# dkohlsdorf/audio_pattern_discovery

Hardware: AMD Instinct MI355X
Metric: DTW cell-updates/sec (whole node) (higher is better)
Workload: dtype f32

## Files before the change

### audio_pattern_discovery_amd/csrc/apd_api.hip

```cpp
#include <algorithm>
#include <cmath>
#include <cstdio>
#include <cstdlib>
#include <cstring>
#include <map>
#include <new>

#include "apd_internal.h"

using namespace apd;

namespace {

int ensure_ws(apd_context *ctx, void **p, size_t *have, size_t need)
{
    APD_AFFINITY(ctx, "workspace allocation");
    if (*have >= need && *p) return APD_OK;
    if (*p) { HIP_TRY(ctx, hipFree(*p)); *p = nullptr; *have = 0; }
    HIP_TRY(ctx, hipMalloc(p, need));
    *have = need;
    return APD_OK;
}

uint32_t tiles_side(uint32_t n_seq) { return (n_seq + kTile - 1) / kTile; }
// ... 43 lines not shown
    return hipSetDevice(ctx->device);
}
bool affinity_ok(const apd_context *ctx, const char *where)
{
    int dev = -1;
    const bool ok = tl_bound_context == ctx && hipGetDevice(&dev) == hipSuccess && dev == ctx->device;
    if (!ok) {
        const_cast<apd_context *>(ctx)->last_error = std::string("APD_DEBUG_AFFINITY: ") + where + " on a thread bound to " +
            (tl_bound_context == ctx ? "this context but HIP device " + std::to_string(dev) :
             tl_bound_context ? "another context (device " + std::to_string(tl_bound_context->device) + ")" : "no context") +
            ", expected device " + std::to_string(ctx->device);
        std::fprintf(stderr, "[apd] %s\n", ctx->last_error.c_str());
    }
    return ok;
}
}


extern "C" const char *apd_status_string(int s)
{
    switch (s) {
        case APD_OK: return "ok";
        case APD_ERR_INVALID_ARG: return "invalid argument";
        case APD_ERR_NO_DEVICE: return "no gfx950 HIP device";
        case APD_ERR_HIP: return "HIP runtime error";
        case APD_ERR_OOM: return "out of device memory";
        case APD_ERR_EMPTY_SEQUENCE: return "zero-length sequence (undefined in the reference, alignments.rs:120)";
        case APD_ERR_BAND_TOO_WIDE: return "warping band too wide for one wavefront";
        case APD_ERR_INDEX: return "percentile index out of range (the reference panics, numerics.rs:132)";
        case APD_ERR_UNSUPPORTED: return "unsupported";
        case APD_ERR_INCOMPLETE: return "a pair score was never written (launch cut short or skipped): NaN left in the output";
        case APD_ERR_COMM: return "RCCL error";
        default: return "unknown status";
    }
}

extern "C" int apd_create(int device, apd_context **out)
{
    if (!out) return APD_ERR_INVALID_ARG;
    *out = nullptr;
    int count = 0;
    if (hipGetDeviceCount(&count) != hipSuccess || count <= 0 || device < 0 || device >= count) return APD_ERR_NO_DEVICE;
    hipDeviceProp_t prop;
    if (hipGetDeviceProperties(&prop, device) != hipSuccess) return APD_ERR_NO_DEVICE;
    if (std::strncmp(prop.gcnArchName, "gfx950", 6) != 0) return APD_ERR_NO_DEVICE;
    apd_context *ctx = new (std::nothrow) apd_context();
    if (!ctx) return APD_ERR_OOM;
    ctx->device = device;
    if (bind_device(ctx) != hipSuccess || hipStreamCreateWithFlags(&ctx->stream, hipStreamNonBlocking) != hipSuccess) {
        delete ctx;
        return APD_ERR_HIP;
    }
    ctx->own_stream = true;
    if (hipMalloc((void **)&ctx->d_status, 64) != hipSuccess || hipMemset(ctx->d_status, 0, 64) != hipSuccess) {
        hipStreamDestroy(ctx->stream);
        delete ctx;
        return APD_ERR_OOM;
    }
    hipEventCreate(&ctx->ev0);
    hipEventCreate(&ctx->ev1);
    hipEventCreateWithFlags(&ctx->fork, hipEventDisableTiming);
    for (int k = 0; k < apd_context::kSideStreams; ++k) {
        hipStreamCreateWithFlags(&ctx->side[k], hipStreamNonBlocking);
        hipEventCreateWithFlags(&ctx->side_done[k], hipEventDisableTiming);
    }
    *out = ctx;
    return APD_OK;
}

static void release_batch_device_memory(apd_batch *b);

extern "C" int apd_destroy(apd_context *ctx)
{
    if (!ctx) return APD_ERR_INVALID_ARG;
    bind_device(ctx);
    hipStreamSynchronize(ctx->stream);
    if (ctx->pair_batch) { apd_batch_destroy(ctx->pair_batch); ctx->pair_batch = nullptr; }
    for (apd_batch *b : ctx->batches) { release_batch_device_memory(b); b->ctx = nullptr; }
    ctx->batches.clear();
    for (apd_comm *c : ctx->comms) apd::orphan_comm(c);
    ctx->comms.clear();
    for (apd_encoder *e : ctx->encoders) apd::orphan_encoder(e);
    ctx->encoders.clear();
    for (apd_cepstrum_plan *cp : ctx->cepstrum_plans) apd::orphan_cepstrum_plan(cp);
    ctx->cepstrum_plans.clear();
    for (void *p : ctx->buffers) hipFree(p);
    ctx->buffers.clear();
    if (ctx->ws_tiles) hipFree(ctx->ws_tiles);
    if (ctx->ws_slab) hipFree(ctx->ws_slab);
    if (ctx->ws_misc) hipFree(ctx->ws_misc);
    if (ctx->ws_gather) hipFree(ctx->ws_gather);
    if (ctx->d_status) hipFree(ctx->d_status);
    if (ctx->ev0) hipEventDestroy(ctx->ev0);
    if (ctx->ev1) hipEventDestroy(ctx->ev1);
    if (ctx->fork) hipEventDestroy(ctx->fork);
    for (int k = 0; k < apd_context::kSideStreams; ++k) {
        if (ctx->side[k]) { hipStreamSynchronize(ctx->side[k]); hipStreamDestroy(ctx->side[k]); }
        if (ctx->side_done[k]) hipEventDestroy(ctx->side_done[k]);
    }
    if (ctx->own_stream && ctx->stream) hipStreamDestroy(ctx->stream);
    delete ctx;
    return APD_OK;
}

extern "C" int apd_set_stream(apd_context *ctx, void *hip_stream)
{
// ... 296 lines not shown
extern "C" int apd_length_order(const uint64_t *offsets, uint32_t n_seq, uint32_t *order)
{
    if (!offsets || (n_seq && !order)) return APD_ERR_INVALID_ARG;
    std::vector<uint32_t> o;
    length_order(offsets, n_seq, o);
    std::copy(o.begin(), o.end(), order);
    return APD_OK;
}

extern "C" int apd_unpack_tiles_host(const uint64_t *offsets, uint32_t n_seq, uint32_t world, const float *gathered, float *out)
{
    if (!offsets || world == 0 || (n_seq && (!gathered || !out))) return APD_ERR_INVALID_ARG;
    std::vector<uint32_t> order;
    length_order(offsets, n_seq, order);
    const uint64_t slab = apd_slab_floats(n_seq, world);
    std::memset(out, 0, (size_t)n_seq * n_seq * sizeof(float));
    const uint32_t side = tiles_side(n_seq);
    uint64_t g = 0;
    for (uint32_t ta = 0; ta < side; ++ta)
        for (uint32_t tb = ta; tb < side; ++tb, ++g) {
            const float *t = gathered + (g % world) * slab + (g / world) * 2 * kSlotsPerTile;
            for (uint32_t sa = 0; sa < kTile; ++sa)
                for (uint32_t sb = 0; sb < kTile; ++sb) {
                    const uint32_t pa = ta * kTile + sa, pb = tb * kTile + sb;
                    if (pa < pb && pb < n_seq) {
                        const uint32_t a = order[pa], b = order[pb];
                        out[(uint64_t)a * n_seq + b] = t[sa * kTile + sb];
                        out[(uint64_t)b * n_seq + a] = t[kSlotsPerTile + sa * kTile + sb];
                    }
                }
        }
    return APD_OK;
}

static int check_lengths(const apd_batch *b)
{
    if (b->n_seq > 0 && b->min_len == 0) return APD_ERR_EMPTY_SEQUENCE;
    return APD_OK;
}

static int build_tile_plan(apd_context *ctx, const apd_batch *batch, const BandSpec &band, uint32_t rank, uint32_t world,
                           bool fast_ok, bool uniform_pen, bool fast_shift, apd_batch::TilePlan &plan_out)
{
    apd_batch::TilePlan plan;
    std::vector<uint2> tiles;
    rank_tile_list(batch->n_seq, rank, world, tiles);
    std::vector<uint4> flat;
    plan_tile_classes(batch->offsets, batch->n_seq, tiles, band, batch->dim, ctx->variant, fast_ok, uniform_pen, fast_shift,
                      plan.classes, flat);
    if (std::getenv("APD_DEBUG_PLAN"))
        for (const TileClass &tc : plan.classes)
            std::fprintf(stderr, "[apd] rank %u/%u: geometry %d: %u tiles, w_max %u, n_max %u\n", rank, world, tc.geom.encode(), tc.count,
                         tc.w_max, tc.n_max);
    HIP_TRY(ctx, hipMalloc((void **)&plan.d_tiles, std::max<size_t>(flat.size(), 1) * sizeof(uint4)));
    if (!flat.empty()) {
        hipError_t e = hipMemcpyAsync(plan.d_tiles, flat.data(), flat.size() * sizeof(uint4), hipMemcpyHostToDevice, ctx->stream);
        if (e == hipSuccess) e = hipStreamSynchronize(ctx->stream);
        if (e != hipSuccess) {
            hipFree(plan.d_tiles);
            ctx->last_error = std::string("tile plan upload: ") + hipGetErrorString(e);
            return APD_ERR_HIP;
        }
    }
    plan_out = std::move(plan);
    return APD_OK;
}

static int align_tiles_impl(apd_context *ctx, const apd_batch *batch, const BandSpec &band, uint32_t rank,
                            uint32_t world, float *d_slab)
{
    if (!ctx || !batch || !d_slab || world == 0 || rank >= world || batch->ctx != ctx) return APD_ERR_INVALID_ARG;
    int rc = check_lengths(batch);
    if (rc) return rc;
    HIP_TRY(ctx, bind_device(ctx));
    const bool pens_ok = (band.ins > 0.0f) && (band.del > 0.0f) && (band.mat > 0.0f) && (band.ins < INFINITY) &&
                         (band.del < INFINITY) && (band.mat < INFINITY);
    const bool static_fast = pens_ok && batch->frames_bytes != 0;
    bool nonfinite = false, device_select = false;
    if (static_fast) {
        const uint32_t band_ub = band.use_explicit ? band.explicit_band : host_band_from_pct(band.pct, batch->max_len);
        const uint32_t w_all = std::max(std::min(band_ub, batch->max_len), batch->max_len - batch->min_len) + 2;
        device_select = generic_fallback_fits(w_all) && apd_num_tiles(batch->n_seq) * kSlotsPerTile <= 0xFFFFFFFFull;
        if (!device_select) {
            rc = batch_nonfinite(ctx, batch, &nonfinite);
            if (rc) return rc;
        }
    }
    const bool fast_ok = static_fast && !nonfinite;
    const bool strict = ctx->distance_mode == 2;
    const bool uniform_pen = (band.ins == band.del) && (band.del == band.mat) && !strict;
    char keybuf[160];
    uint32_t pct_bits;
    std::memcpy(&pct_bits, &band.pct, sizeof(pct_bits));
    const bool fast_shift = band.ins == 1.0f && band.del == 1.0f && band.mat == 1.0f && ctx->distance_mode == 1 && batch->dim >= 8;
    std::snprintf(keybuf, sizeof(keybuf), "%u/%u/%08x/%u/%d/%d/%d/%d/%d", rank, world, pct_bits, band.explicit_band, band.use_explicit,
                  ctx->variant, (int)fast_ok, (int)uniform_pen, (int)fast_shift);
    auto cached = batch->tile_cache.find(keybuf);
    if (cached == batch->tile_cache.end()) {
        apd_batch::TilePlan fresh;
        rc = build_tile_plan(ctx, batch, band, rank, world, fast_ok, uniform_pen, fast_shift, fresh);
        if (rc) return rc;
        cached = batch->tile_cache.emplace(keybuf, std::move(fresh)).first;
    }
    const apd_batch::TilePlan &plan = cached->second;
    APD_AFFINITY(ctx, "alignment launches");
    HIP_TRY(ctx, hipMemsetAsync(d_slab, 0xFF, apd_slab_floats(batch->n_seq, world) * sizeof(float), ctx->stream));
    AlignLaunch L{};
    L.d_frames = batch->d_frames; L.frames_bytes = batch->frames_bytes; L.d_seq_off = batch->d_seq_off; L.d_seq_nmax = batch->d_seq_nmax;
    L.n_seq = batch->n_seq; L.dim = batch->dim; L.dpad = batch->dpad; L.band = band; L.d_slab = d_slab;
    L.variant = ctx->variant;
    L.hybrid = ctx->distance_mode == 1; L.strict = strict; L.tau = ctx->tau;
    L.d_nonfinite = device_select ? batch->d_flags : nullptr;
    if (ctx->timing) HIP_TRY(ctx, hipEventRecord(ctx->ev0, ctx->stream));
    const bool fan_out = plan.classes.size() > 1 && ctx->side[0] != nullptr;
    if (fan_out) {
        HIP_TRY(ctx, hipEventRecord(ctx->fork, ctx->stream));
        for (int k = 0; k < apd_context::kSideStreams; ++k) HIP_TRY(ctx, hipStreamWaitEvent(ctx->side[k], ctx->fork, 0));
    }
    int rc_launch = APD_OK;
    size_t ci = 0;
    for (const TileClass &tc : plan.classes) {
        L.d_tiles = plan.d_tiles + tc.first; L.n_tiles = tc.count; L.w_max = tc.w_max; L.n_max = tc.n_max;
        if (ctx->drop_tiles) L.n_tiles -= std::min(L.n_tiles, ctx->drop_tiles);
        int status = APD_OK;
        hipStream_t s = fan_out ? ctx->side[ci++ % apd_context::kSideStreams] : ctx->stream;
        hipError_t e = launch_align(L, tc.geom, s, ctx->last_error, &status);
        if (e != hipSuccess) { ctx->last_error = std::string("launch_align: ") + hipGetErrorString(e); rc_launch = APD_ERR_HIP; break; }
        if (status != APD_OK) { rc_launch = status; break; }
    }
    if (fan_out)
        for (int k = 0; k < apd_context::kSideStreams; ++k) {
            HIP_TRY(ctx, hipEventRecord(ctx->side_done[k], ctx->side[k]));
            HIP_TRY(ctx, hipStreamWaitEvent(ctx->stream, ctx->side_done[k], 0));
        }
    if (rc_launch != APD_OK) return rc_launch;
    if (device_select) {
        size_t k = 0;
        while (k < plan.classes.size()) {
            if (plan.classes[k].geom.family == KernelGeom::Generic) { ++k; continue; }
            uint32_t first = plan.classes[k].first, total = 0, w_max = 0, n_max = 0;
            for (; k < plan.classes.size() && plan.classes[k].geom.family != KernelGeom::Generic && plan.classes[k].first == first + total; ++k) {
                total += plan.classes[k].count; w_max = std::max(w_max, plan.classes[k].w_max); n_max = std::max(n_max, plan.classes[k].n_max);
            }
            L.d_tiles = plan.d_tiles + first; L.n_tiles = total; L.w_max = w_max; L.n_max = n_max;
            if (ctx->drop_tiles) L.n_tiles -= std::min(L.n_tiles, ctx->drop_tiles);
            bool fits = true;
            const hipError_t e = launch_generic_fallback(L, ctx->stream, &fits);
            if (e != hipSuccess || !fits) { ctx->last_error = std::string("launch_generic_fallback: ") + (fits ? hipGetErrorString(e) : "band too wide"); return APD_ERR_HIP; }
        }
    }
    if (ctx->timing) { HIP_TRY(ctx, hipEventRecord(ctx->ev1, ctx->stream)); ctx->timed = true; }
    return APD_OK;
}

static BandSpec band_from_cfg(const apd_align_config *cfg)
{
    BandSpec b{};
    b.pct = cfg->warping_band_percentage; b.use_explicit = 0; b.explicit_band = 0;
    b.ins = cfg->insertion_penalty; b.del = cfg->deletion_penalty; b.mat = cfg->match_penalty;
    return b;
}

extern "C" int apd_align_tiles_async(apd_context *ctx, const apd_batch *batch, const apd_align_config *cfg,
                                     uint32_t rank, uint32_t world, float *d_slab)
{
    if (!cfg) return APD_ERR_INVALID_ARG;
    return align_tiles_impl(ctx, batch, band_from_cfg(cfg), rank, world, d_slab);
}

extern "C" int apd_unpack_tiles_async(apd_context *ctx, const apd_batch *batch, uint32_t world, const float *d_gathered,
                                      float *d_out)
{
    if (!ctx || !batch || batch->ctx != ctx || !d_gathered || !d_out || world == 0) return APD_ERR_INVALID_ARG;
    const uint32_t n_seq = batch->n_seq;
    HIP_TRY(ctx, bind_device(ctx));
    APD_AFFINITY(ctx, "unpack launch");
    HIP_TRY(ctx, hipMemsetAsync(d_out, 0xFF, (size_t)n_seq * n_seq * sizeof(float), ctx->stream));
    HIP_TRY(ctx, launch_unpack(d_gathered, d_out, batch->d_order, n_seq, world, apd_slab_floats(n_seq, world), batch->d_flags,
                               ctx->d_status, ctx->stream));
    return APD_OK;
}

static int align_all_device_impl(apd_context *ctx, const apd_batch *batch, const BandSpec &band, float *d_out)
{
    if (!ctx || !batch || !d_out) return APD_ERR_INVALID_ARG;
    const size_t slab_bytes = std::max<size_t>(apd_slab_floats(batch->n_seq, 1) * sizeof(float), 16);
    int rc = ensure_ws(ctx, &ctx->ws_slab, &ctx->ws_slab_bytes, slab_bytes);
    if (rc) return rc;
// ... 153 lines not shown
```

### audio_pattern_discovery_amd/csrc/apd_internal.h

```cpp
#pragma once
#include <hip/hip_runtime.h>
#include <stdint.h>

#include <iterator>
#include <map>
#include <set>
#include <string>
#include <type_traits>
#include <utility>
#include <vector>

#include "../../include/apd.h"

struct apd_context;
namespace apd {

constexpr int kTile = 16;
constexpr int kSlotsPerTile = kTile * kTile;
constexpr int kWave = 64;

struct BandSpec {
    float pct;
    uint32_t explicit_band;
    int use_explicit;
    float ins, del, mat;
};

struct AlignLaunch {
    const float *d_frames;
    uint32_t frames_bytes;
    const uint32_t *d_seq_off;
    const float *d_seq_nmax;
    const uint4 *d_tiles;
    uint32_t n_tiles;
    uint32_t n_seq;
    uint32_t dim, dpad;
    BandSpec band;
    float *d_slab;
    const uint32_t *d_nonfinite;
    uint32_t w_max;
    uint32_t n_max;
    int variant;
    int hybrid;
    int strict;
    float tau;
};

constexpr int kKernelDims[] = {8, 10, 13, 16, 20, 26};
constexpr bool is_kernel_dim(uint32_t d) { for (int k : kKernelDims) if ((uint32_t)k == d) return true; return false; }
constexpr uint32_t kernel_dim(uint32_t d) { for (int k : kKernelDims) if ((uint32_t)k >= d) return (uint32_t)k; return d; }
constexpr int max_cells_per_lane(uint32_t d) { return d <= 13 ? 9 : (d <= 16 ? 7 : 5); }
constexpr int max_strip_columns(uint32_t d) { return d <= 10 ? 13 : (d <= 13 ? 11 : max_cells_per_lane(d)); }

struct KernelGeom {
    enum Family : uint8_t { Generic, Systolic, Wide, Strip, BandedStrip };
    Family family = Generic;
    uint8_t lanes_or_waves = 0;
    uint8_t cells = 0;

    constexpr int encode() const
    {
        constexpr int base[] = {0, 0, 10000, 20000, 30000};
        return family == Generic ? 0 : base[family] + lanes_or_waves * 100 + cells;
    }
    static constexpr KernelGeom decode(int key)
    {
        const Family f = key >= 100 && key < 10000 ? Systolic : key >= 10000 && key < 20000 ? Wide
                       : key >= 20000 && key < 30000 ? Strip : key >= 30000 && key < 40000 ? BandedStrip : Generic;
        if (f == Generic) return KernelGeom{};
        return KernelGeom{f, (uint8_t)((key % 10000) / 100), (uint8_t)(key % 100)};
    }
    constexpr uint32_t lanes_per_pair() const
    {
        return family == Systolic ? lanes_or_waves : family == Wide ? 64u * lanes_or_waves : 64u;
    }
    constexpr uint32_t capacity() const { return (family == Wide ? 64u : 1u) * lanes_or_waves * cells; }
    constexpr bool operator==(KernelGeom o) const { return family == o.family && lanes_or_waves == o.lanes_or_waves && cells == o.cells; }
    constexpr bool operator<(KernelGeom o) const { return encode() < o.encode(); }
};

#define APD_SYSTOLIC_GEOMS(X) X(8, 5) X(8, 7) X(8, 9) X(16, 2) X(16, 3) X(16, 5) X(16, 7) X(16, 9) X(32, 5) X(32, 7) X(32, 9) \
                              X(64, 3) X(64, 5) X(64, 7) X(64, 9)
#define APD_WIDE_GEOMS(X) X(2, 5) X(2, 7) X(2, 9) X(4, 5) X(4, 7) X(4, 9) X(8, 5) X(8, 7) X(8, 9)
#define APD_STRIP_GEOMS(X) X(1, 3) X(1, 5) X(1, 7) X(1, 9) X(1, 11) X(1, 13) X(2, 3) X(2, 5) X(2, 7) X(2, 9) X(2, 11) X(2, 13) \
                           X(4, 3) X(4, 5) X(4, 7) X(4, 9) X(4, 11) X(4, 13)
#define APD_BANDED_STRIP_GEOMS(X) X(1, 5) X(1, 9) X(4, 5) X(4, 9)

#define APD_SYSTOLIC_ENTRY_(A, B) KernelGeom{KernelGeom::Systolic, A, B},
#define APD_WIDE_ENTRY_(A, B) KernelGeom{KernelGeom::Wide, A, B},
#define APD_STRIP_ENTRY_(A, B) KernelGeom{KernelGeom::Strip, A, B},
#define APD_BANDED_STRIP_ENTRY_(A, B) KernelGeom{KernelGeom::BandedStrip, A, B},
constexpr KernelGeom kSystolicGeoms[] = {APD_SYSTOLIC_GEOMS(APD_SYSTOLIC_ENTRY_)};
// ... 64 lines not shown

inline uint32_t host_band_from_pct(float pct, uint32_t len)
{
    float p = pct * (float)len;
    if (!(p > 0.0f)) return 0;
    if (p >= 4294967040.0f) return 0xFFFFFFFFu;
    return (uint32_t)p;
}
inline uint32_t host_w(const BandSpec &b, uint32_t n, uint32_t m)
{
    uint32_t mx = n > m ? n : m, gap = n > m ? n - m : m - n;
    uint32_t band = b.use_explicit ? b.explicit_band : host_band_from_pct(b.pct, mx);
    if (band > mx) band = mx;
    return (band > gap ? band : gap) + 2;
}

extern thread_local const apd_context *tl_bound_context;
bool affinity_debug();
hipError_t bind_device(const apd_context *ctx);
bool affinity_ok(const apd_context *ctx, const char *where);

}

#define APD_AFFINITY(ctx, where)                                                                   \
    do { if (apd::affinity_debug() && !apd::affinity_ok((ctx), (where))) return APD_ERR_HIP; } while (0)

#define HIP_TRY(ctx, call)                                                             \
    do {                                                                               \
        if (hipError_t e_ = (call); e_ != hipSuccess) {                                \
            (ctx)->last_error = std::string(#call) + ": " + hipGetErrorString(e_);     \
            return e_ == hipErrorOutOfMemory ? APD_ERR_OOM : APD_ERR_HIP;              \
        }                                                                              \
    } while (0)

struct apd_context {
    int device = 0;
    hipStream_t stream = nullptr;
    bool own_stream = false;
    bool timing = false;
    hipEvent_t ev0 = nullptr, ev1 = nullptr;
    static constexpr int kSideStreams = 4;
    hipStream_t side[kSideStreams] = {nullptr, nullptr, nullptr, nullptr};
    hipEvent_t side_done[kSideStreams] = {nullptr, nullptr, nullptr, nullptr};
    hipEvent_t fork = nullptr;
    std::set<apd_batch *> batches;
    std::set<apd_comm *> comms;
    std::set<apd_encoder *> encoders;
    std::set<apd_cepstrum_plan *> cepstrum_plans;
    std::set<void *> buffers;
    bool timed = false;
    int variant = 0;
    int distance_mode = 1;
    float tau = 1.0f / 64.0f;
    std::string last_error;
    void *ws_tiles = nullptr; size_t ws_tiles_bytes = 0;
    void *ws_slab = nullptr; size_t ws_slab_bytes = 0;
    void *ws_misc = nullptr; size_t ws_misc_bytes = 0;
    void *ws_gather = nullptr; size_t ws_gather_bytes = 0;
    uint32_t *d_status = nullptr;
    uint32_t drop_tiles = 0;
    apd_batch *pair_batch = nullptr;
    uint64_t pair_n = 0, pair_m = 0;
    uint32_t pair_dim = 0;
};

struct apd_batch {
    apd_context *ctx = nullptr;
    uint32_t n_seq = 0, dim = 0, dpad = 0;
    uint32_t src_dim = 0;
    uint64_t total_frames = 0;
    float *d_frames = nullptr;
    uint32_t frames_bytes = 0;
    uint32_t *d_meta = nullptr;
    std::vector<uint32_t> h_meta;
    uint32_t *d_seq_off = nullptr;
    uint32_t *d_src_off = nullptr;
    uint32_t *d_order = nullptr;
    uint32_t *d_flags = nullptr;
    float *d_seq_nmax = nullptr;
    mutable int nonfinite = -1;
    std::vector<uint32_t> order;
    std::vector<uint64_t> offsets;
    uint32_t min_len = 0, max_len = 0;
    struct TilePlan { uint4 *d_tiles = nullptr; std::vector<apd::TileClass> classes; };
    mutable std::map<std::string, TilePlan> tile_cache;
};
```

### audio_pattern_discovery_amd/csrc/dtw_generic.hip

```cpp
#include <algorithm>
#include <cmath>
#include <type_traits>
#include "dtw_common.h"

namespace apd {

__device__ __forceinline__ void generic_pair(const AlignLaunch &L, int c_max, uint32_t wave, float *lds)
{
    const int lane = threadIdx.x;
    const uint32_t tile = wave / kSlotsPerTile, slot = wave % kSlotsPerTile;
    const PairInfo P = decode_pair(L, tile, slot);
    if (!P.valid) return;
    const int n = P.n, m = P.m, w = P.w;
    if (n == 1 || m == 1) {
        if (lane == 0) { const float s = (n == 1 && m == 1) ? 0.0f : APD_INF; store_pair(L, tile, P, s, s); }
        return;
    }
    const float ins = L.band.ins, del = L.band.del, mat = L.band.mat;
    const int two_w = 2 * w;
    int C = (two_w + 1 + 63) / 64;
    C = max(C, 2);
    float *p1 = lds, *p2 = lds + c_max * 64;
    for (int c = 0; c < C; ++c) { p1[c * 64 + lane] = APD_INF; p2[c * 64 + lane] = APD_INF; }
    const int dp4 = (int)L.dpad / 4, dim = (int)L.dim;
// ... 385 lines not shown
        classes.push_back(TileClass{g.first, (uint32_t)flat.size(), (uint32_t)g.second.tiles.size(), g.second.w_max, g.second.n_max});
        flat.insert(flat.end(), g.second.tiles.begin(), g.second.tiles.end());
    }
}

static size_t generic_lds_bytes(uint32_t w_max, int *c_max_out)
{
    int c_max = (int)((2 * (uint64_t)w_max + 1 + 63) / 64);
    if (c_max < 2) c_max = 2;
    if (c_max_out) *c_max_out = c_max;
    return (size_t)c_max * 64 * 2 * sizeof(float);
}

static hipError_t launch_align_chunk(const AlignLaunch &L, KernelGeom g, hipStream_t stream, std::string &err, int *status)
{
    if (L.n_tiles == 0) return hipSuccess;
    if (g.family == KernelGeom::Generic) {
        int c_max = 2;
        const size_t lds_bytes = generic_lds_bytes(L.w_max, &c_max);
        if (lds_bytes > 160 * 1024) { *status = APD_ERR_BAND_TOO_WIDE; err = "band too wide for the generic kernel"; return hipSuccess; }
        if (lds_bytes > 64 * 1024) {
            hipError_t e = hipFuncSetAttribute(reinterpret_cast<const void *>(dtw_fused_generic),
                                               hipFuncAttributeMaxDynamicSharedMemorySize, (int)lds_bytes);
            if (e != hipSuccess) return e;
        }
        const uint64_t waves = (uint64_t)L.n_tiles * kSlotsPerTile;
        hipLaunchKernelGGL(dtw_fused_generic, dim3((uint32_t)waves), dim3(64), lds_bytes, stream, L, c_max);
        return hipGetLastError();
    }
    hipError_t e = hipSuccess;
    bool found = false;
    with_kernel_dim(L.dim, [&](auto d) {
        constexpr int D = decltype(d)::value;
        found = g.family == KernelGeom::Systolic ? launch_systolic<D>(L, g, stream)
              : g.family == KernelGeom::Wide     ? launch_wide<D>(L, g, stream, &e)
                                                 : launch_full<D>(L, g, stream, &e);
    });
    if (!found) {
        *status = APD_ERR_UNSUPPORTED;
        err = "no kernel for geometry " + std::to_string(g.encode()) + " at dimension " + std::to_string(L.dim);
        return hipSuccess;
    }
    return e != hipSuccess ? e : hipGetLastError();
}

hipError_t launch_align(const AlignLaunch &L, KernelGeom g, hipStream_t stream, std::string &err, int *status)
{
    *status = APD_OK;
    const uint32_t kTilesPerLaunch = (1u << 31) / (kSlotsPerTile * std::max(g.lanes_per_pair(), 64u));
    AlignLaunch part = L;
    part.hybrid = L.hybrid && (g.family == KernelGeom::Systolic ? L.dim >= 8 && !L.strict : L.dim >= 10 && L.band.mat == 1.0f);
    for (uint32_t first = 0; first < L.n_tiles; first += kTilesPerLaunch) {
        part.d_tiles = L.d_tiles + first;
        part.n_tiles = std::min(kTilesPerLaunch, L.n_tiles - first);
        const hipError_t e = launch_align_chunk(part, g, stream, err, status);
        if (e != hipSuccess || *status != APD_OK) return e;
    }
    return hipSuccess;
}

bool generic_fallback_fits(uint32_t w_max)
{
    const size_t lds_bytes = generic_lds_bytes(w_max, nullptr);
    if (lds_bytes > 160 * 1024) return false;
    if (lds_bytes > 64 * 1024 &&
        hipFuncSetAttribute(reinterpret_cast<const void *>(dtw_fused_generic_fallback), hipFuncAttributeMaxDynamicSharedMemorySize,
                            (int)lds_bytes) != hipSuccess) {
        (void)hipGetLastError();
        return false;
    }
    return true;
}

hipError_t launch_generic_fallback(const AlignLaunch &L, hipStream_t stream, bool *fits)
{
    *fits = true;
    if (L.n_tiles == 0 || L.d_nonfinite == nullptr) return hipSuccess;
    int c_max = 2;
    const size_t lds_bytes = generic_lds_bytes(L.w_max, &c_max);
    if (lds_bytes > 160 * 1024) { *fits = false; return hipSuccess; }
    if (lds_bytes > 64 * 1024) {
        hipError_t e = hipFuncSetAttribute(reinterpret_cast<const void *>(dtw_fused_generic_fallback),
                                           hipFuncAttributeMaxDynamicSharedMemorySize, (int)lds_bytes);
        if (e != hipSuccess) return e;
    }
    const uint64_t waves = (uint64_t)L.n_tiles * kSlotsPerTile;
    if (waves > 0xFFFFFFFFull) { *fits = false; return hipSuccess; }
    const uint32_t grid = (uint32_t)std::min<uint64_t>(waves, 256u * 32u);
    hipLaunchKernelGGL(dtw_fused_generic_fallback, dim3(grid), dim3(64), lds_bytes, stream, L, c_max, (uint32_t)waves);
    return hipGetLastError();
}

}
```

### audio_pattern_discovery_amd/csrc/dtw_systolic.h

```cpp
#pragma once
#include <type_traits>

#ifndef APD_ABLATE
#define APD_ABLATE 0
#endif

#include "dtw_common.h"

namespace apd {

typedef float apd_f32x4 __attribute__((ext_vector_type(4)));
constexpr uint32_t kNoFrame = 0xFFFFFF00u;

template <int D>
__device__ __forceinline__ void load_frame(float (&dst)[D], __amdgpu_buffer_rsrc_t rsrc, uint32_t byte_off)
{
    constexpr int DP4 = (D + 3) / 4;
#pragma unroll
    for (int q = 0; q < DP4; ++q) {
        const apd_f32x4 t = __builtin_bit_cast(apd_f32x4, __builtin_amdgcn_raw_buffer_load_b128(rsrc, byte_off + 16u * q, 0, 0));
        if (4 * q + 0 < D) dst[4 * q + 0] = t.x;
        if (4 * q + 1 < D) dst[4 * q + 1] = t.y;
        if (4 * q + 2 < D) dst[4 * q + 2] = t.z;
        if (4 * q + 3 < D) dst[4 * q + 3] = t.w;
// ... 20 lines not shown
    }
    if (APD_ABLATE & 1) return acc;
    return __builtin_amdgcn_sqrtf(acc);
}

template <int D, int DN>
__device__ __forceinline__ float frame_sq_strict(const float (&x)[DN], const float (&y)[DN])
{
    float t = x[0] - y[0];
    float acc = t * t;
#pragma unroll
    for (int k = 1; k < D; ++k) {
        t = x[k] - y[k];
        const float sq = t * t;
        acc = acc + sq;
    }
    return acc;
}
template <int D, int DN>
__device__ __forceinline__ float frame_dist_strict(const float (&x)[DN], const float (&y)[DN])
{
    return __builtin_sqrtf(frame_sq_strict<D, DN>(x, y));
}

template <int D>
__device__ __forceinline__ float frame_sq_expanded_pre(const float (&xm)[D + 1], const float (&y)[D + 1])
{
    float acc = xm[D] + y[D];
#pragma unroll
    for (int k = 0; k < D; ++k) acc = __builtin_fmaf(xm[k], y[k], acc);
    return acc;
}
template <int D>
__device__ __forceinline__ void prescale_row_piece(apd_f32x4 &v, int piece)
{
    const bool np = piece == D / 4;
    v.x = (np && D % 4 == 0) ? v.x : -2.0f * v.x;
    v.y = (np && D % 4 == 1) ? v.y : -2.0f * v.y;
    v.z = (np && D % 4 == 2) ? v.z : -2.0f * v.z;
    v.w = (np && D % 4 == 3) ? v.w : -2.0f * v.w;
}
template <int D>
__device__ __forceinline__ float frame_sq_exact_pre(const float (&xm)[D + 1], const float (&y)[D + 1])
{
    float t = __builtin_fmaf(-0.5f, xm[0], -y[0]);
    float acc = t * t;
#pragma unroll
    for (int k = 1; k < D; ++k) {
        t = __builtin_fmaf(-0.5f, xm[k], -y[k]);
        acc = __builtin_fmaf(t, t, acc);
    }
    return acc;
}
template <int D, int C, int G, bool UNIFORM_PEN, bool HYBRID>
__global__ __launch_bounds__(256) void dtw_fused_systolic(const AlignLaunch L)
{
    static_assert(C >= 2 && (64 % G) == 0, "bad geometry");
    if (L.d_nonfinite != nullptr && *L.d_nonfinite != 0u) return;
    constexpr int DN = D + 1;
    constexpr int DP = (DN + 3) & ~3;
    constexpr int PPW = 64 / G;
    constexpr int WPT = kSlotsPerTile / (4 * PPW);
    const int lane = threadIdx.x & 63;
    const int gl = lane % G;
    const uint32_t xcd = blockIdx.x & 7u, q = blockIdx.x >> 3;
    const uint32_t tile = (q / WPT) * 8u + xcd;
    const uint32_t slot = ((q % WPT) * 4u + (threadIdx.x >> 6)) * PPW + lane / G;
    const PairInfo P = decode_pair(L, tile, slot);
    const bool special = P.valid && (P.n == 1 || P.m == 1);
    const bool sweep = P.valid && !special;
    if (__ballot(sweep) == 0ull) {
        if (special && gl == 0) { const float s = (P.n == 1 && P.m == 1) ? 0.0f : APD_INF; store_pair(L, tile, P, s, s); }
        return;
    }
    const int n = sweep ? P.n : 1, m = sweep ? P.m : 1, w = sweep ? P.w : 2;
    const __amdgpu_buffer_rsrc_t rsrc = __builtin_amdgcn_make_buffer_rsrc((void *)L.d_frames, 0, L.frames_bytes, 0x00020000);
    const uint32_t a_off = (uint32_t)(P.A - L.d_frames) * 4u, b_off = (uint32_t)(P.B - L.d_frames) * 4u;
    constexpr uint32_t FB = DP * 4u;
    float ins = L.band.ins, del = L.band.del, mat = L.band.mat;
    float tau_thr = L.tau, nmax_b = P.nmax_b;
    asm volatile("" : "+v"(ins), "+v"(del), "+v"(mat), "+v"(tau_thr), "+v"(nmax_b));
    constexpr int R = (G == 64) ? 128 : 64;
    constexpr int LPF = DP / 4;
    constexpr int FPF = 64 / LPF;
    constexpr int RS = DP + 4;
    constexpr int U_ROWS = ((C + 1) % 2 == 0) ? (C + 1) : 2 * (C + 1);
    __shared__ float xring_all[4][(R + U_ROWS) * RS];
    float *const xring = xring_all[threadIdx.x >> 6];
    const int lead = __builtin_ctzll(__ballot(sweep));
    const uint32_t a_off_w = __builtin_amdgcn_readlane(a_off, lead);
    const int n_w = __builtin_amdgcn_readlane(n, lead);
    const int u0 = C * gl;
    const int two_w = 2 * w;

    bool g1[C], g2[C];
#pragma unroll
    for (int c = 0; c < C; ++c) {
        const int u = u0 + c;
        g1[c] = u >= two_w;
        g2[c] = (u == 0) | (u > two_w);
    }
    const int cw = w - u0;
    const int ustar = (m - 1) - (n - 1) + w;
    const int cstar = ustar - u0;
    const int tau_cap = (n - 1) + gl;

    const int g_act = (two_w + 1 + C - 1) / C;
    int my_total = sweep ? (n - 1) + g_act : 0;
    int my_min = sweep ? (n - 1) : 0x7fffffff;
    int total = 0, min_rows = 0x7fffffff;
#pragma unroll
    for (int g = 0; g < PPW; ++g) {
        total = max(total, __builtin_amdgcn_readlane(my_total, g * G));
        min_rows = min(min_rows, __builtin_amdgcn_readlane(my_min, g * G));
    }
    constexpr int S = C + 1;
    constexpr int U = (S % 2 == 0) ? S : 2 * S;
    static_assert(U == U_ROWS, "ring copy sized for another unroll");
    constexpr bool MASKED_FETCH = HYBRID && (G == 32 || G == 8) && !(APD_ABLATE & 512);
    const int total_r = ((total + U - 1) / U) * U;
    int a_steps = G;
    if (UNIFORM_PEN && !HYBRID) {
        int w_max = 0;
#pragma unroll
        for (int g = 0; g < PPW; ++g) w_max = max(w_max, __builtin_amdgcn_readlane(w, g * G));
        a_steps = max(G, w_max + 1);
    }
    const int a_end = min(((a_steps + U - 1) / U) * U, total_r);
    const int b_end = min(max((min_rows / U) * U, a_end), total_r);

    float prev1[C], prev2[C];
#pragma unroll
    for (int c = 0; c < C; ++c) { prev1[c] = APD_INF; prev2[c] = APD_INF; }
    float res1 = 0.0f, res2 = 0.0f;

    float yf[S][DN];
#pragma unroll
    for (int c = 0; c < C; ++c) {
        const int j = u0 - gl + c - w;
        const int idx = (j >= 1) ? (min(j, m) - 1) : (HYBRID ? m : m + 1);
        load_frame<DN>(yf[c], rsrc, b_off + (uint32_t)idx * FB);
// ... 31 lines not shown
    };
    for (int e = lane; e < G * DP; e += 64) {
        const int slot = (-(e / DP)) & (R - 1);
        const float v = HYBRID ? ((e % DP) == D ? APD_INF : 0.0f) : -APD_INF;
        xring[slot * RS + (e % DP)] = v;
        if (slot < U) xring[(slot + R) * RS + (e % DP)] = v;
    }
    {
        apd_f32x4 regs[NFILL];
        fill_load(1, regs);
        fill_store(1, regs);
    }
    asm volatile("" ::: "memory");
    auto read_row = [&](float (&dst)[DN], int row) __attribute__((always_inline)) {
        const float *p = &xring[(row & (R - 1)) * RS];
#pragma unroll
        for (int q = 0; q < LPF; ++q) {
            const apd_f32x4 t = *reinterpret_cast<const apd_f32x4 *>(p + 4 * q);
            if (4 * q + 0 < DN) dst[4 * q + 0] = t.x;
            if (4 * q + 1 < DN) dst[4 * q + 1] = t.y;
            if (4 * q + 2 < DN) dst[4 * q + 2] = t.z;
            if (4 * q + 3 < DN) dst[4 * q + 3] = t.w;
        }
    };
    auto read_row_at = [&](float (&dst)[DN], const float *p) __attribute__((always_inline)) {
#pragma unroll
        for (int q = 0; q < LPF; ++q) {
            const apd_f32x4 t = *reinterpret_cast<const apd_f32x4 *>(p + 4 * q);
            if (4 * q + 0 < DN) dst[4 * q + 0] = t.x;
            if (4 * q + 1 < DN) dst[4 * q + 1] = t.y;
            if (4 * q + 2 < DN) dst[4 * q + 2] = t.z;
            if (4 * q + 3 < DN) dst[4 * q + 3] = t.w;
        }
    };
    constexpr int NX = HYBRID ? 1 : 2;
    float xs[NX][DN];
    read_row(xs[0], 0 - gl);
#pragma unroll
    for (int k = 0; k < DN; ++k) xs[NX - 1][k] = (NX == 1) ? xs[0][k] : 0.0f;
    constexpr bool PIPE = (APD_ABLATE & 32) != 0;
    float dn[C];
#pragma unroll
    for (int c = 0; c < C; ++c) dn[c] = (PIPE && !HYBRID && c < C - 1) ? frame_dist_strict<D, DN>(xs[0], yf[c]) : 0.0f;

    auto advance_window = [&](int q) __attribute__((always_inline)) {
        const int r = q % S, e = (r + C) % S;
#pragma unroll
        for (int k = 0; k < (HYBRID ? DN : D); ++k) {
            if (APD_ABLATE & 4) { yf[e][k] = yf[(r + 1) % S][k] + yf[e][k]; continue; }
            yf[e][k] = MASKED_FETCH ? dpp_move<(G == 8) ? 0x101 : 0x130>(yf[(r + 1) % S][k], yf[e][k])
                                    : group_from_upper<G>(yf[(r + 1) % S][k], yf[e][k], gl);
        }
    };
    auto macro_steps = [&](int tau_begin, int tau_end, auto slow_tag) __attribute__((always_inline)) {
        constexpr bool SLOW = decltype(slow_tag)::value;
        uint32_t yo_cur = kNoFrame, yo_cap = kNoFrame, yo_step = 0u;
        if (!SLOW && gl == G - 1) {
            yo_cap = b_off + (uint32_t)(m - 1) * FB;
            yo_cur = min(b_off + (uint32_t)(tau_begin + ((HYBRID && !MASKED_FETCH) ? 1 : 0) + (C - 1) * G - w) * FB, yo_cap);
            yo_step = FB;
        }
        auto fetch_column = [&](float (&dst)[DN], int t) __attribute__((always_inline)) {
            if (APD_ABLATE & 8) return;
            if (SLOW) {
                const int jt = t + 1 + (C - 1) * G - w;
                const uint32_t yo = b_off + (uint32_t)((jt >= 1) ? (min(jt, m) - 1) : (HYBRID ? m : m + 1)) * FB;
                load_frame<DN>(dst, rsrc, gl == G - 1 ? yo : kNoFrame);
            } else {
                load_frame<DN>(dst, rsrc, yo_cur);
                yo_cur = min(yo_cur + yo_step, yo_cap);
            }
        };
        for (int tau0 = tau_begin; tau0 < tau_end; tau0 += U) {
            apd_f32x4 fill_regs[NFILL];
            fill_load(tau0 + U + 1, fill_regs);
            const float *const xrows = &xring[((tau0 + 1 - gl) & (R - 1)) * RS];
#pragma unroll
            for (int q = 0; q < U; ++q) {
                const int tau = tau0 + q;
                const int r = q % S;
                const int xa = HYBRID ? 0 : (q & 1), xb = HYBRID ? 0 : (xa ^ 1);
                const int e = (r + C) % S;
                if (!HYBRID) {
                    fetch_column(yf[e], tau);
                    read_row_at(xs[xb], xrows + q * RS);
                }
                float d[C];
                if (HYBRID) {
#pragma unroll
                    for (int c = 0; c < C; ++c) {
                        d[c] = frame_sq_expanded_pre<D>(xs[xa], yf[(r + c) % S]);
                    }
                    float dmin = d[0];
#pragma unroll
                    for (int c = 1; c + 1 < C; c += 2) dmin = __builtin_fminf(__builtin_fminf(dmin, d[c]), d[c + 1]);
                    if (C % 2 == 0) dmin = __builtin_fminf(dmin, d[C - 1]);
                    const bool any = (APD_ABLATE & 128) ? false : dmin < (xs[xa][D] + nmax_b) * tau_thr;
                    advance_window(q);
                    if (MASKED_FETCH) {
                        if (gl == G - 1) fetch_column(yf[e], tau);
                    }
                    if (__builtin_expect(__ballot(any) != 0ull, 0)) {
                        float nx = xs[xa][D];
                        asm volatile("" : "+v"(nx));
#pragma unroll
                        for (int c = 0; c < C; ++c) {
                            const float sc = nx + yf[(r + c) % S][D];
                            const float ex = frame_sq_exact_pre<D>(xs[xa], yf[(r + c) % S]);
                            d[c] = (d[c] < sc * tau_thr) ? ex : d[c];
                        }
                    }
                    if (!MASKED_FETCH) fetch_column(yf[r], tau + 1);
#pragma unroll
                    for (int c = 0; c < C; ++c) d[c] = (APD_ABLATE & 1) ? d[c] : __builtin_amdgcn_sqrtf(d[c]);
                    read_row_at(xs[0], xrows + q * RS);
                } else if (UNIFORM_PEN && !SLOW && !PIPE) {
                    float d2[C];
#pragma unroll
                    for (int c = 0; c < C; ++c) d2[c] = frame_sq_strict<D, DN>(xs[xa], yf[(r + c) % S]);
                    float dmin = d2[0];
#pragma unroll
                    for (int c = 1; c + 1 < C; c += 2) dmin = __builtin_fminf(__builtin_fminf(dmin, d2[c]), d2[c + 1]);
                    if (C % 2 == 0) dmin = __builtin_fminf(dmin, d2[C - 1]);
                    if (__builtin_expect(__ballot(!(dmin >= 0x1p-96f)) != 0ull, 0)) {
#pragma unroll
                        for (int c = 0; c < C; ++c) d[c] = __builtin_sqrtf(d2[c]);
                    } else {
#pragma unroll
                        for (int c = 0; c < C; ++c) d[c] = sqrt_rn_finite(d2[c]);
                    }
                } else {
#pragma unroll
                    for (int c = 0; c < C; ++c)
                        d[c] = (UNIFORM_PEN && PIPE && c < C - 1) ? dn[c] : frame_dist_strict<D, DN>(xs[xa], yf[(r + c) % S]);
                    if (PIPE) {
#pragma unroll
                        for (int c = 0; c < C - 1; ++c) dn[c] = frame_dist_strict<D, DN>(xs[xb], yf[(r + 1 + c) % S]);
                    }
                }
                float left1 = group_from_lower_wrap<G>(prev1[C - 1], APD_INF, gl);
                float left2 = group_from_lower_wrap<G>(prev2[C - 1], APD_INF, gl);
                float upr1 = APD_INF, upr2 = APD_INF;
#pragma unroll
                for (int c = 0; c < C; ++c) {
                    if (APD_ABLATE & 2) { prev1[c] += d[c]; prev2[c] -= d[c]; continue; }
                    const float up1 = (c < C - 1) ? prev1[(c + 1) % C] : upr1;
                    const float up2 = (c < C - 1) ? prev2[(c + 1) % C] : upr2;
                    const float r1 = select_node<UNIFORM_PEN>(left1, up1, prev1[c], d[c], del, ins, mat, (APD_ABLATE & 16) ? false : g1[c]);
                    const float r2 = select_node<UNIFORM_PEN>(up2, left2, prev2[c], d[c], del, ins, mat, (APD_ABLATE & 16) ? false : g2[c]);
                    prev1[c] = r1; prev2[c] = r2;
                    left1 = r1; left2 = r2;
                    if (c == 0) {
                        upr1 = group_from_upper_wrap<G>(r1, APD_INF, gl);
                        upr2 = group_from_upper_wrap<G>(r2, APD_INF, gl);
                    }
                }
                if (SLOW) {
                    if (tau == gl) {
#pragma unroll
                        for (int c = 0; c < C; ++c) if (c == cw) { prev1[c] = 0.0f; prev2[c] = 0.0f; }
                    }
                    if (tau == tau_cap) {
#pragma unroll
                        for (int c = 0; c < C; ++c) if (c == cstar) { res1 = prev1[c]; res2 = prev2[c]; }
                    }
                }
                if (!HYBRID) advance_window(q);
            }
            fill_store(tau0 + U + 1, fill_regs);
            asm volatile("" ::: "memory");
        }
    };
    macro_steps(0, a_end, std::true_type{});
    macro_steps(a_end, b_end, std::false_type{});
    macro_steps(b_end, total_r, std::true_type{});

    if (P.valid && gl == (sweep ? ustar / C : 0)) {
        if (sweep) {
            const float denom = (float)(n + m);
            store_pair(L, tile, P, res1 / denom, res2 / denom);
        } else {
            const float s = (P.n == 1 && P.m == 1) ? 0.0f : APD_INF;
            store_pair(L, tile, P, s, s);
        }
    }
}

template <int D, int C, int G, bool UNIFORM_PEN, bool HYBRID>
static void launch_systolic_kernel(const AlignLaunch &L, hipStream_t stream)
{
    constexpr int PPW = 64 / G;
    constexpr int WPT = kSlotsPerTile / (4 * PPW);
    const uint32_t tiles8 = (L.n_tiles + 7u) / 8u * 8u;
    hipLaunchKernelGGL((dtw_fused_systolic<D, C, G, UNIFORM_PEN, HYBRID>), dim3(tiles8 * WPT), dim3(256), 0, stream, L);
}

#ifdef APD_SYSTOLIC_STRICT_UNIT
template <int D>
bool launch_systolic_strict(const AlignLaunch &L, KernelGeom g, hipStream_t stream)
{
#define APD_CASE(GG, CC) if constexpr (geom_instantiated(KernelGeom{KernelGeom::Systolic, GG, CC}, D)) { \
        if (g == KernelGeom{KernelGeom::Systolic, GG, CC}) { launch_systolic_kernel<D, CC, GG, true, false>(L, stream); return true; } }
    APD_SYSTOLIC_GEOMS(APD_CASE)
#undef APD_CASE
    return false;
}
#else
template <int D>
bool launch_systolic(const AlignLaunch &L, KernelGeom g, hipStream_t stream)
{
    const bool unit = L.band.ins == 1.0f && L.band.del == 1.0f && L.band.mat == 1.0f;
    if (unit && !L.hybrid) return launch_systolic_strict<D>(L, g, stream);
#define APD_CASE(GG, CC) if constexpr (geom_instantiated(KernelGeom{KernelGeom::Systolic, GG, CC}, D)) { \
        if (g == KernelGeom{KernelGeom::Systolic, GG, CC}) { \
            if (!unit) launch_systolic_kernel<D, CC, GG, false, false>(L, stream); else launch_systolic_kernel<D, CC, GG, true, true>(L, stream); \
            return true; } }
    APD_SYSTOLIC_GEOMS(APD_CASE)
#undef APD_CASE
    return false;
}
#endif

}
```

Baseline: 2911 billion.

## Defer hybrid exact-distance fallback to a second pass over marked wavefronts

In hybrid distance mode, the systolic kernel no longer runs the rare exact-distance branch inline. Each wavefront ORs its ballot, abandons the sweep as soon as any lane needs the exact path, and sets a bit in a per-tile mark array. A second persistent kernel then reruns only the marked wavefronts with the full branch. This removes the divergent fallback code from the hot loop, which can lower register pressure and branch overhead. The cost is an extra memset, an extra launch, and redone work for every flagged wavefront.

```diff
diff --git a/audio_pattern_discovery_amd/csrc/apd_api.hip b/audio_pattern_discovery_amd/csrc/apd_api.hip
--- a/audio_pattern_discovery_amd/csrc/apd_api.hip
+++ b/audio_pattern_discovery_amd/csrc/apd_api.hip
@@ -119,6 +119,7 @@
         return APD_ERR_HIP;
     }
     ctx->own_stream = true;
+    if (const char *v = std::getenv("APD_HYBRID_DEFER")) ctx->hybrid_defer = !(v[0] == '0' && v[1] == '\0');
     if (hipMalloc((void **)&ctx->d_status, 64) != hipSuccess || hipMemset(ctx->d_status, 0, 64) != hipSuccess) {
         hipStreamDestroy(ctx->stream);
         delete ctx;
@@ -521,7 +522,9 @@
         for (const TileClass &tc : plan.classes)
             std::fprintf(stderr, "[apd] rank %u/%u: geometry %d: %u tiles, w_max %u, n_max %u\n", rank, world, tc.geom.encode(), tc.count,
                          tc.w_max, tc.n_max);
-    HIP_TRY(ctx, hipMalloc((void **)&plan.d_tiles, std::max<size_t>(flat.size(), 1) * sizeof(uint4)));
+    plan.n_tiles = flat.size();
+    HIP_TRY(ctx, hipMalloc((void **)&plan.d_tiles, std::max<size_t>(flat.size(), 1) * (sizeof(uint4) + kSlotsPerTile / 8)));
+    plan.d_marks = reinterpret_cast<uint32_t *>(plan.d_tiles + std::max<size_t>(flat.size(), 1));
     if (!flat.empty()) {
         hipError_t e = hipMemcpyAsync(plan.d_tiles, flat.data(), flat.size() * sizeof(uint4), hipMemcpyHostToDevice, ctx->stream);
         if (e == hipSuccess) e = hipStreamSynchronize(ctx->stream);
@@ -574,6 +577,8 @@
     const apd_batch::TilePlan &plan = cached->second;
     APD_AFFINITY(ctx, "alignment launches");
     HIP_TRY(ctx, hipMemsetAsync(d_slab, 0xFF, apd_slab_floats(batch->n_seq, world) * sizeof(float), ctx->stream));
+    const bool defer = ctx->hybrid_defer && ctx->distance_mode == 1 && plan.n_tiles > 0;
+    if (defer) HIP_TRY(ctx, hipMemsetAsync(plan.d_marks, 0, plan.n_tiles * (kSlotsPerTile / 8), ctx->stream));
     AlignLaunch L{};
     L.d_frames = batch->d_frames; L.frames_bytes = batch->frames_bytes; L.d_seq_off = batch->d_seq_off; L.d_seq_nmax = batch->d_seq_nmax;
     L.n_seq = batch->n_seq; L.dim = batch->dim; L.dpad = batch->dpad; L.band = band; L.d_slab = d_slab;
@@ -590,6 +595,7 @@
     size_t ci = 0;
     for (const TileClass &tc : plan.classes) {
         L.d_tiles = plan.d_tiles + tc.first; L.n_tiles = tc.count; L.w_max = tc.w_max; L.n_max = tc.n_max;
+        L.d_marks = defer ? plan.d_marks + (size_t)tc.first * (kSlotsPerTile / 32) : nullptr;
         if (ctx->drop_tiles) L.n_tiles -= std::min(L.n_tiles, ctx->drop_tiles);
         int status = APD_OK;
         hipStream_t s = fan_out ? ctx->side[ci++ % apd_context::kSideStreams] : ctx->stream;
@@ -603,6 +609,20 @@
             HIP_TRY(ctx, hipStreamWaitEvent(ctx->stream, ctx->side_done[k], 0));
         }
     if (rc_launch != APD_OK) return rc_launch;
+    L.d_marks = nullptr;
+    if (defer && std::getenv("APD_DEBUG_MARKS")) {
+        std::vector<uint32_t> marks(plan.n_tiles * (kSlotsPerTile / 32));
+        HIP_TRY(ctx, hipMemcpyAsync(marks.data(), plan.d_marks, marks.size() * sizeof(uint32_t), hipMemcpyDeviceToHost, ctx->stream));
+        HIP_TRY(ctx, hipStreamSynchronize(ctx->stream));
+        for (const TileClass &tc : plan.classes) {
+            if (tc.geom.family != KernelGeom::Systolic) continue;
+            uint64_t bits = 0;
+            for (size_t k = (size_t)tc.first * (kSlotsPerTile / 32); k < ((size_t)tc.first + tc.count) * (kSlotsPerTile / 32); ++k) bits += (uint64_t)__builtin_popcount(marks[k]);
+            const uint64_t ppw = 64 / tc.geom.lanes_or_waves, waves = (uint64_t)tc.count * kSlotsPerTile / ppw;
+            std::fprintf(stderr, "[apd] rank %u/%u: geometry %d: %llu of %llu wavefronts marked (%.4f %%)\n", rank, world, tc.geom.encode(),
+                         (unsigned long long)(bits / ppw), (unsigned long long)waves, waves ? 100.0 * (double)(bits / ppw) / (double)waves : 0.0);
+        }
+    }
     if (device_select) {
         size_t k = 0;
         while (k < plan.classes.size()) {
diff --git a/audio_pattern_discovery_amd/csrc/apd_internal.h b/audio_pattern_discovery_amd/csrc/apd_internal.h
--- a/audio_pattern_discovery_amd/csrc/apd_internal.h
+++ b/audio_pattern_discovery_amd/csrc/apd_internal.h
@@ -38,6 +38,7 @@
     BandSpec band;
     float *d_slab;
     const uint32_t *d_nonfinite;
+    uint32_t *d_marks;
     uint32_t w_max;
     uint32_t n_max;
     int variant;
@@ -208,6 +209,7 @@
     int variant = 0;
     int distance_mode = 1;
     float tau = 1.0f / 64.0f;
+    bool hybrid_defer = true;
     std::string last_error;
     void *ws_tiles = nullptr; size_t ws_tiles_bytes = 0;
     void *ws_slab = nullptr; size_t ws_slab_bytes = 0;
@@ -238,6 +240,6 @@
     std::vector<uint32_t> order;
     std::vector<uint64_t> offsets;
     uint32_t min_len = 0, max_len = 0;
-    struct TilePlan { uint4 *d_tiles = nullptr; std::vector<apd::TileClass> classes; };
+    struct TilePlan { uint4 *d_tiles = nullptr; uint32_t *d_marks = nullptr; size_t n_tiles = 0; std::vector<apd::TileClass> classes; };
     mutable std::map<std::string, TilePlan> tile_cache;
 };
diff --git a/audio_pattern_discovery_amd/csrc/dtw_generic.hip b/audio_pattern_discovery_amd/csrc/dtw_generic.hip
--- a/audio_pattern_discovery_amd/csrc/dtw_generic.hip
+++ b/audio_pattern_discovery_amd/csrc/dtw_generic.hip
@@ -461,6 +461,7 @@
     part.hybrid = L.hybrid && (g.family == KernelGeom::Systolic ? L.dim >= 8 && !L.strict : L.dim >= 10 && L.band.mat == 1.0f);
     for (uint32_t first = 0; first < L.n_tiles; first += kTilesPerLaunch) {
         part.d_tiles = L.d_tiles + first;
+        part.d_marks = L.d_marks ? L.d_marks + (size_t)first * (kSlotsPerTile / 32) : nullptr;
         part.n_tiles = std::min(kTilesPerLaunch, L.n_tiles - first);
         const hipError_t e = launch_align_chunk(part, g, stream, err, status);
         if (e != hipSuccess || *status != APD_OK) return e;
diff --git a/audio_pattern_discovery_amd/csrc/dtw_systolic.h b/audio_pattern_discovery_amd/csrc/dtw_systolic.h
--- a/audio_pattern_discovery_amd/csrc/dtw_systolic.h
+++ b/audio_pattern_discovery_amd/csrc/dtw_systolic.h
@@ -96,20 +96,19 @@
     }
     return acc;
 }
-template <int D, int C, int G, bool UNIFORM_PEN, bool HYBRID>
-__global__ __launch_bounds__(256) void dtw_fused_systolic(const AlignLaunch L)
-{
-    static_assert(C >= 2 && (64 % G) == 0, "bad geometry");
-    if (L.d_nonfinite != nullptr && *L.d_nonfinite != 0u) return;
+enum SweepMode : int { Immediate = 0, Deferred = 1, Marked = 2 };
+constexpr int kMarkWordsPerTile = kSlotsPerTile / 32;
+
+template <int D, int C, int G, bool UNIFORM_PEN, bool HYBRID, int MODE>
+__device__ __forceinline__ void systolic_sweep(const AlignLaunch &L, const uint32_t tile, const uint32_t slot0, float *const xring)
+{
     constexpr int DN = D + 1;
     constexpr int DP = (DN + 3) & ~3;
     constexpr int PPW = 64 / G;
-    constexpr int WPT = kSlotsPerTile / (4 * PPW);
-    const int lane = threadIdx.x & 63;
+    int lane = threadIdx.x & 63;
+    if (MODE == Marked) asm volatile("" : "+v"(lane));
     const int gl = lane % G;
-    const uint32_t xcd = blockIdx.x & 7u, q = blockIdx.x >> 3;
-    const uint32_t tile = (q / WPT) * 8u + xcd;
-    const uint32_t slot = ((q % WPT) * 4u + (threadIdx.x >> 6)) * PPW + lane / G;
+    const uint32_t slot = slot0 + lane / G;
     const PairInfo P = decode_pair(L, tile, slot);
     const bool special = P.valid && (P.n == 1 || P.m == 1);
     const bool sweep = P.valid && !special;
@@ -129,8 +128,6 @@
     constexpr int FPF = 64 / LPF;
     constexpr int RS = DP + 4;
     constexpr int U_ROWS = ((C + 1) % 2 == 0) ? (C + 1) : 2 * (C + 1);
-    __shared__ float xring_all[4][(R + U_ROWS) * RS];
-    float *const xring = xring_all[threadIdx.x >> 6];
     const int lead = __builtin_ctzll(__ballot(sweep));
     const uint32_t a_off_w = __builtin_amdgcn_readlane(a_off, lead);
     const int n_w = __builtin_amdgcn_readlane(n, lead);
@@ -268,7 +265,8 @@
                                     : group_from_upper<G>(yf[(r + 1) % S][k], yf[e][k], gl);
         }
     };
-    auto macro_steps = [&](int tau_begin, int tau_end, auto slow_tag) __attribute__((always_inline)) {
+    unsigned long long flagged = 0ull;
+    auto macro_steps = [&](int tau_begin, int tau_end, auto slow_tag) __attribute__((always_inline)) -> bool {
         constexpr bool SLOW = decltype(slow_tag)::value;
         uint32_t yo_cur = kNoFrame, yo_cap = kNoFrame, yo_step = 0u;
         if (!SLOW && gl == G - 1) {
@@ -316,7 +314,9 @@
                     if (MASKED_FETCH) {
                         if (gl == G - 1) fetch_column(yf[e], tau);
                     }
-                    if (__builtin_expect(__ballot(any) != 0ull, 0)) {
+                    if (MODE == Deferred) {
+                        flagged |= __ballot(any);
+                    } else if (__builtin_expect(__ballot(any) != 0ull, 0)) {
                         float nx = xs[xa][D];
                         asm volatile("" : "+v"(nx));
 #pragma unroll
@@ -385,11 +385,16 @@
             }
             fill_store(tau0 + U + 1, fill_regs);
             asm volatile("" ::: "memory");
-        }
-    };
-    macro_steps(0, a_end, std::true_type{});
-    macro_steps(a_end, b_end, std::false_type{});
-    macro_steps(b_end, total_r, std::true_type{});
+            if (MODE == Deferred && flagged != 0ull) return true;
+        }
+        return false;
+    };
+    const bool stop = macro_steps(0, a_end, std::true_type{}) || macro_steps(a_end, b_end, std::false_type{}) ||
+                      macro_steps(b_end, total_r, std::true_type{});
+    if (MODE == Deferred && stop) {
+        if (lane == 0) atomicOr(&L.d_marks[tile * kMarkWordsPerTile + (slot0 >> 5)], ((1u << PPW) - 1u) << (slot0 & 31u));
+        return;
+    }
 
     if (P.valid && gl == (sweep ? ustar / C : 0)) {
         if (sweep) {
@@ -402,13 +407,63 @@
     }
 }
 
-template <int D, int C, int G, bool UNIFORM_PEN, bool HYBRID>
+template <int D, int C, int G>
+__device__ __forceinline__ float *systolic_ring()
+{
+    constexpr int DP = (D + 1 + 3) & ~3;
+    constexpr int R = (G == 64) ? 128 : 64, RS = DP + 4, U_ROWS = ((C + 1) % 2 == 0) ? (C + 1) : 2 * (C + 1);
+    __shared__ float xring_all[4][(R + U_ROWS) * RS];
+    return xring_all[threadIdx.x >> 6];
+}
+
+template <int D, int C, int G, bool UNIFORM_PEN, bool HYBRID, int MODE>
+__global__ __launch_bounds__(256) void dtw_fused_systolic(const AlignLaunch L)
+{
+    static_assert(C >= 2 && (64 % G) == 0, "bad geometry");
+    static_assert(MODE == Immediate || (MODE == Deferred && UNIFORM_PEN && HYBRID), "only the hybrid form has a test to defer");
+    if (L.d_nonfinite != nullptr && *L.d_nonfinite != 0u) return;
+    constexpr int PPW = 64 / G;
+    constexpr int WPT = kSlotsPerTile / (4 * PPW);
+    const uint32_t xcd = blockIdx.x & 7u, q = blockIdx.x >> 3;
+    const uint32_t tile = (q / WPT) * 8u + xcd;
+    systolic_sweep<D, C, G, UNIFORM_PEN, HYBRID, MODE>(L, tile, ((q % WPT) * 4u + (threadIdx.x >> 6)) * PPW, systolic_ring<D, C, G>());
+}
+
+template <int D, int C, int G>
+__global__ __launch_bounds__(256, 2) void dtw_fused_systolic_marked(const AlignLaunch L)
+{
+    if (L.d_nonfinite != nullptr && *L.d_nonfinite != 0u) return;
+    constexpr int PPW = 64 / G;
+    float *const xring = systolic_ring<D, C, G>();
+    const uint32_t n_waves = gridDim.x * 4u;
+    const uint32_t wave = blockIdx.x * 4u + __builtin_amdgcn_readfirstlane(threadIdx.x >> 6);
+    for (uint32_t item = wave; item < L.n_tiles * kMarkWordsPerTile; item += n_waves) {
+        for (uint32_t bits = __builtin_amdgcn_readfirstlane(L.d_marks[item]); bits != 0u;) {
+            const uint32_t first = (uint32_t)__builtin_ctz(bits) & ~(uint32_t)(PPW - 1);
+            bits &= ~(((1u << PPW) - 1u) << first);
+            asm volatile("" ::: "memory");
+            systolic_sweep<D, C, G, true, true, Marked>(L, item / kMarkWordsPerTile, (item % kMarkWordsPerTile) * 32u + first, xring);
+        }
+    }
+}
+
+template <int D, int C, int G, bool UNIFORM_PEN, bool HYBRID, int MODE = Immediate>
 static void launch_systolic_kernel(const AlignLaunch &L, hipStream_t stream)
 {
     constexpr int PPW = 64 / G;
     constexpr int WPT = kSlotsPerTile / (4 * PPW);
     const uint32_t tiles8 = (L.n_tiles + 7u) / 8u * 8u;
-    hipLaunchKernelGGL((dtw_fused_systolic<D, C, G, UNIFORM_PEN, HYBRID>), dim3(tiles8 * WPT), dim3(256), 0, stream, L);
+    if constexpr (MODE == Marked)
+        hipLaunchKernelGGL((dtw_fused_systolic_marked<D, C, G>), dim3(std::min(L.n_tiles * (kMarkWordsPerTile / 4u), 512u)), dim3(256), 0, stream, L);
+    else
+        hipLaunchKernelGGL((dtw_fused_systolic<D, C, G, UNIFORM_PEN, HYBRID, MODE>), dim3(tiles8 * WPT), dim3(256), 0, stream, L);
+}
+template <int D, int C, int G>
+static void launch_systolic_hybrid(const AlignLaunch &L, hipStream_t stream)
+{
+    if (L.d_marks == nullptr) { launch_systolic_kernel<D, C, G, true, true, Immediate>(L, stream); return; }
+    launch_systolic_kernel<D, C, G, true, true, Deferred>(L, stream);
+    launch_systolic_kernel<D, C, G, true, true, Marked>(L, stream);
 }
 
 #ifdef APD_SYSTOLIC_STRICT_UNIT
@@ -429,7 +484,7 @@
     if (unit && !L.hybrid) return launch_systolic_strict<D>(L, g, stream);
 #define APD_CASE(GG, CC) if constexpr (geom_instantiated(KernelGeom{KernelGeom::Systolic, GG, CC}, D)) { \
         if (g == KernelGeom{KernelGeom::Systolic, GG, CC}) { \
-            if (!unit) launch_systolic_kernel<D, CC, GG, false, false>(L, stream); else launch_systolic_kernel<D, CC, GG, true, true>(L, stream); \
+            if (!unit) launch_systolic_kernel<D, CC, GG, false, false>(L, stream); else launch_systolic_hybrid<D, CC, GG>(L, stream); \
             return true; } }
     APD_SYSTOLIC_GEOMS(APD_CASE)
 #undef APD_CASE
```

Result: slower. 2624 billion (-9.9%).
